# jamesli1618/Obj-GAN

Measured on AMD Instinct MI355X. Metric: G+D train-step images/sec at 256x256, batch 16 per GPU, higher is better.
Workload: dtype fp32 (fp16x2: operands as two fp16 pieces of x * 2^s on the fp16 MFMA); 1 GPU; stage3_256x256_full_GD_step: RNN_ENCODER+G_NET(3 stages)+PatD x3+ShpD x3+ObjSSD+ObjLSD(ROIAlign)+DAMSM+KL+Adam x9+EMA+IS-monitor; per_gpu_batch=16, global_batch=16, parallelism=dp1, fresh_batch_every_step=True

## Files before the change

### include/objgan_hip.h

```cpp
#ifndef OBJGAN_HIP_H
#define OBJGAN_HIP_H

#ifdef __cplusplus
extern "C" {
#endif

int objgan_roi_align_forward(const float* features, const float* rois, float* output,
                             int num_rois, int roi_cols, int channels, int height, int width,
                             int aligned_height, int aligned_width, float spatial_scale,
                             void* stream);
int objgan_roi_align_backward(const float* top_grad, const float* rois, float* bottom_grad,
                              int batch_size, int num_rois, int roi_cols, int channels,
                              int height, int width, int aligned_height, int aligned_width,
                              float spatial_scale, void* stream);

long objgan_roi_align_backward_ws_floats(int batch_size, int num_rois, int channels, int height, int width,
                                         int aligned_height, int aligned_width);
int objgan_roi_align_backward_ordered(const float* top_grad, const float* rois, float* bottom_grad,
                                      int batch_size, int num_rois, int roi_cols, int channels,
                                      int height, int width, int aligned_height, int aligned_width,
                                      float spatial_scale, float* ws, long ws_floats, void* stream);
int objgan_avgpool2s1_forward(const float* in, float* out, long planes, int ih, int iw, void* stream);
int objgan_avgpool2s1_backward(const float* grad_out, float* grad_in, long planes, int ih, int iw,
                               void* stream);

long objgan_conv_packed_floats(int M, int C, int T);
int objgan_conv_bank_layout(int N, int C, int H, int W, int M, int Tg, int PH, int PW, int act, int math);
int objgan_conv_igemm(const float* x, const float* w, const float* bias, float* y, float* wt,
                      int N, int C, int H, int W, int upsample, int pad_mode,
                      int Cout, int Cin, int Torig, int transpose,
                      int Tg, const int* dh, const int* dw, const int* src_tap,
                      int PH, int PW, int stride,
                      int OHf, int OWf, int osh, int osw, int ooh, int oow,
                      int act, int y_prezeroed, int wt_packed, int math, float* ring, const float* xmax, float* ymax,
                      float* ws, long ws_floats, void* stream);
int objgan_absmax_partials(const float* x, long n, float* out1024, void* stream);
long objgan_h2_records_floats(int N, int C, long HW);
int objgan_h2_records(const float* x, const float* xmax1024, void* rec, int N, int C, long HW, void* stream);
long objgan_conv_igemm_ws_floats(int N, int C, int H, int W, int upsample, int pad_mode,
                                 int Cout, int Cin, int Torig, int transpose, int Tg,
                                 int PH, int PW, int stride, int OHf, int OWf, int osh, int osw,
                                 int act, int y_prezeroed, int math, int ring);
int objgan_reflect_ring_fold(const float* ring, float* y, long planes, int H, int W, void* stream);
long objgan_conv_dgrad_s2_phases_ws_floats(int N, int Cout, int OH, int OW, int math);
long objgan_conv_dgrad_s2_thin_floats(int Cout, int Cin);
int objgan_conv_pack_job_thin_phase(void* job, const float* w, float* wt, int Cout, int Cin, int phase);
int objgan_conv_dgrad_s2_thin(const float* dy, const float* w, float* dx, float* wt, int N, int Cout, int OH, int OW,
                              int Cin, int wt_packed, void* stream);
int objgan_conv_dgrad_s2_phases(const float* x, const float* w, float* y, float* wt,
                                int N, int Cout, int OH, int OW, int Cin, int Torig,
                                int Tg, const int* dh, const int* dw, const int* src_tap,
                                int PH, int PW, int wt_packed, int math, const float* xmax, float* ws, long ws_floats,
                                void* stream);
long objgan_conv_wgrad_ws_floats(int N, int Cin, int H, int W, int upsample, int pad_mode,
                                 int Cout, int OH, int OW, int ksize, int stride, int pad, int math);
int objgan_conv_wgrad(const float* x, const float* dy, float* dw,
                      int N, int Cin, int H, int W, int upsample, int pad_mode,
                      int Cout, int OH, int OW, int ksize, int stride, int pad, int math,
                      int accumulate, const float* xmax, const float* dymax, float* ws, long ws_floats, void* stream);
int objgan_conv_wgrad_rec_ok(int N, int Cin, int H, int W, int Cout, int OH, int OW, int ksize);
long objgan_nhwc_bf16_floats(int N, int C, long HW);
int objgan_nhwc_bf16(const float* x, float* out, int N, int C, long HW, void* stream);
int objgan_conv_wgrad_bfb_ok(int N, int Cin, int H, int W, int Cout, int OH, int OW, int ksize);

int objgan_lstm_bidir_forward(const float* table, const long* captions, const int* lens,
                              const float* wt_ih, const float* wt_hh, const float* b_ih, const float* b_hh,
                              float* out, float* hn, int B, int L, int Lout, int I, int H, int ntoken,
                              void* stream);

long objgan_norm_ws_floats(int N, int C, int HW, int per_channel);
int objgan_norm_forward(const float* x, float* y, const float* residual,
                        const float* gamma, const float* beta,
                        float* running_mean, float* running_var,
                        float* sums, float* mean, float* rstd,
                        int N, int C, int HW, int per_channel, int mode,
                        float eps, float momentum, float* amax, void* stream);
int objgan_norm_amax_supported(int N, int C, int HW, int per_channel, int affine);
int objgan_norm_apply(const float* x, float* y, const float* residual, const float* gamma, const float* beta,
                      const float* mean, const float* rstd, int N, int C, int HW, int per_channel, int mode,
                      void* stream);
int objgan_norm_backward(const float* x, const float* dy, const float* mean, const float* rstd,
                         const float* gamma, const float* beta, float* bsums,
                         float* dx, float* dgamma, float* dbeta,
                         int N, int C, int HW, int per_channel, int mode, float* amax, void* stream);
int objgan_act_backward(const float* dy, const float* y, float* dz, long total, int kind, float* amax, void* stream);
long objgan_channel_sum_ws_floats(int N, int C, int HW);
int objgan_channel_sum(const float* x, float* out, int N, int C, int HW, float* ws, void* stream);

int objgan_attn_general_forward(const float* x, const float* src, const unsigned char* mask,
                                float* wc, float* attn, int B, int idf, int Q, int L, void* stream);
long objgan_attn_general_backward_ws_floats(int B, int idf, int Q, int L);
int objgan_attn_general_backward(const float* x, const float* src, const float* attn,
                                 const float* dwc, const float* dattn, float* dx, float* dsrc,
                                 int B, int idf, int Q, int L, float* ws, void* stream);
int objgan_attn_bu_forward(const float* tgt, const float* ctx1, const float* src,
                           const unsigned char* mask, float* wc, float* attn,
                           int B, int d2, int idf, int R, int L, int normalize, float eps,
                           void* stream);
int objgan_attn_bu_backward(const float* dwc, const float* attn, float* dsrc,
                            int B, int idf, int R, int L, void* stream);
int objgan_masked_max_forward(const float* f, const float* m, float* out, int B, int num, int R,
                              int P, long m_stride_b, long m_stride_r, long m_stride_c, void* stream);
long objgan_masked_max_backward_ws_floats(int B, int num, int R, int P);
int objgan_masked_max_backward(const float* f, const float* m, const float* dout, float* df,
                               int B, int num, int R, int P, long m_stride_b, long m_stride_r,
                               long m_stride_c, float* ws, void* stream);
int objgan_softmax_strided_forward(const float* x, float* y, long outer, int dim, long inner,
                                   float scale, const int* lens, int nlens,
                                   const unsigned char* rowvalid, void* stream);
int objgan_softmax_strided_backward(const float* y, const float* dy, float* dx, long outer, int dim,
                                    long inner, float scale, void* stream);

int objgan_bilinear_forward(const float* x, float* y, long planes, int ih, int iw, int oh, int ow,
                            void* stream);
int objgan_bilinear_backward(const float* dy, float* dx, long planes, int ih, int iw, int oh, int ow,
                             void* stream);
int objgan_sum2x2(const float* dy, float* dx, long planes, int h, int w, void* stream);
int objgan_reflect_fold(const float* dxp, float* dx, long planes, int h, int w, void* stream);
int objgan_bce_const_forward(const float* p, float* out, int n, float t, void* stream);
int objgan_bce_const_backward(const float* p, const float* g, float* dp, int n, float t, void* stream);
int objgan_conv_pack_job_bytes();
int objgan_conv_pack_job(void* job, const float* w, float* wt, int N, int C, int H, int W, int Cout, int Cin,
                         int Torig, int transpose, int Tg, const int* src_tap, int PH, int PW, int act, int math);
int objgan_conv_pack_job_phase(void* job, const float* w, float* wt, int Cout, int Cin, int Torig, int Tg,
                               const int* src_tap_phase, int phase, int math);
int objgan_conv_pack_jobs_run(const void* jobs_dev, int njobs, void* stream);
int objgan_bmm_strided(const float* A, const float* B, float* C, int batch, int M, int N, int K,
                       long sab, long sam, long sak, long sbb, long sbk, long sbn,
                       long scb, long scm, long scn, void* stream);
int objgan_lift_taps_forward(const float* z, const float* bias, float* y, float* scratch, int N, int Mo, int h,
                             int w, int SH, int SW, const int* ci0, const int* ci1, const float* cl1,
                             const int* ri0, const int* ri1, const float* rl1, void* stream);
int objgan_lift_taps_backward(const float* dy, float* dz, float* scratch, int N, int Mo, int h, int w, int SH,
                              int SW, const int* roff, const int* ridx, const float* rwt, const int* coff,
                              const int* cidx, const float* cwt, void* stream);
int objgan_pool2d_forward(const float* x, float* y, int* idx, long planes, int H, int W, int OH, int OW,
                          int k, int s, int p, int mode, void* stream);
int objgan_pool2d_backward(const float* dy, const int* idx, float* dx, long planes, int H, int W, int OH,
                           int OW, int k, int s, int p, int mode, void* stream);
int objgan_adam_step(float* p, const float* g, float* m, float* v, long n, double lr, double beta1,
                     double beta2, double eps, int step, float grad_scale, void* stream);
int objgan_adam_step_gated(float* p, const float* g, float* m, float* v, long n, double lr, double beta1,
                           double beta2, double eps, double* state, const float* flag, float* coef,
                           float grad_scale, void* stream);
int objgan_ema_update(float* avg, const float* p, long n, float decay, float one_minus_decay,
                      void* stream);

int objgan_resize_pil_kmax(int max_in, int S);
int objgan_resize_pil_rgb8(const unsigned char* src, const long* offs, const int* hs, const int* ws, int B,
                           int Hmax, int kmax, int S, int* coef_scratch, unsigned char* tmp_scratch, float* out,
                           void* stream);

long objgan_jpeg_desc_bytes(void);
long objgan_jpeg_seg_bytes(void);
int objgan_jpeg_parse(const unsigned char* file, long nbytes, void* desc_out);
long objgan_jpeg_plan(void* descs, int n, const long* file_offsets, const long* out_offsets, const int* nsegs);
int objgan_jpeg_decode(const unsigned char* files, const void* descs_host, const void* descs_dev, int n,
                       unsigned char* out, void* ws, long ws_bytes, const void* index_in, void* index_out, void* stream);

int objgan_mask_resize(const double* src, int count, int n, int nsizes, const int* sizes, double* const* out,
                       const int* ntaps, const double* taps, void* stream);

int objgan_bilinear_halfpixel_forward(const float* x, float* y, int N, int C, int H, int W, int OH, int OW,
                                      const float* scale, const float* shift, void* stream);
int objgan_moments_accumulate(const float* x, int rows, int D, double* sum, double* outer, void* stream);
int objgan_moments_finalize(const double* sum, const double* outer, long n, int D, double* mu, double* sigma,
                            void* stream);

long objgan_snapshot_ws_doubles(int nvis, int T, int a, int vis);
int objgan_snapshot_blend_table(unsigned char* table65536);
int objgan_snapshot_grid(const float* imgs, const float* lr_imgs, const float* attn, const int* counts, const double* M,
                         const unsigned char* strip, unsigned char* out, double* ws, long ws_doubles,
                         int nvis, int T, int a, int vis, int H, int W, int LH, int LW,
                         int max_word_num, int font_max, int per_panel_norm, void* stream);

int objgan_prof_enable(int on);
int objgan_prof_collect(double* ms, double* flops, long* count);
int objgan_prof_dump(float* ms, double* flops, int* meta, int max_records, int* n_out);

#ifdef __cplusplus
}
#endif
#endif
```

### obj-gan_amd/csrc/lift_stem.hip

```cpp
#include "common.h"

struct AxisFwd { const int* i0; const int* i1; const float* l1; };
struct AxisBwd { const int* off; const int* idx; const float* wt; };

#define LIFT_MAXE 8

__global__ __launch_bounds__(256) void lift_cols_fwd_kernel(const float* __restrict__ z, float* __restrict__ F,
                                                            long total, int Mo, int h, int w, int SW, AxisFwd t) {
    for (long e = (long)blockIdx.x * blockDim.x + threadIdx.x; e < total; e += (long)gridDim.x * blockDim.x) {
        const int ow = (int)(e % SW);
        long r = e / SW;
        const int qh = (int)(r % h);
        const long n = r / h;
        int i0[3], i1[3];
        float l1[3];
#pragma unroll
        for (int dw = 0; dw < 3; ++dw) { i0[dw] = t.i0[dw * SW + ow]; i1[dw] = t.i1[dw * SW + ow]; l1[dw] = t.l1[dw * SW + ow]; }
        const long hw = (long)h * w;
        const float* zn = z + n * 9 * Mo * hw + (long)qh * w;
        float* Fn = F + (n * 3 * Mo * h + qh) * (long)SW + ow;
        for (int dh = 0; dh < 3; ++dh)
            for (int co = 0; co < Mo; ++co) {
                float acc = 0.f;
#pragma unroll
                for (int dw = 0; dw < 3; ++dw) {
                    const float* zp = zn + ((dh * 3 + dw) * Mo + co) * hw;
                    acc += (1.0f - l1[dw]) * zp[i0[dw]] + l1[dw] * zp[i1[dw]];
                }
                Fn[(long)(dh * Mo + co) * h * SW] = acc;
            }
    }
}

__global__ __launch_bounds__(256) void lift_rows_fwd_kernel(const float* __restrict__ F, const float* __restrict__ bias,
                                                            float* __restrict__ y, long total, int Mo, int h,
                                                            int SH, int SW, AxisFwd t) {
    for (long e = (long)blockIdx.x * blockDim.x + threadIdx.x; e < total; e += (long)gridDim.x * blockDim.x) {
        const int ow = (int)(e % SW);
        long r = e / SW;
        const int oh = (int)(r % SH);
        const long n = r / SH;
        long o0[3], o1[3];
        float l1[3];
#pragma unroll
        for (int dh = 0; dh < 3; ++dh) {
            o0[dh] = (long)t.i0[dh * SH + oh] * SW; o1[dh] = (long)t.i1[dh * SH + oh] * SW; l1[dh] = t.l1[dh * SH + oh];
        }
        const long plane = (long)h * SW;
        const float* Fn = F + n * 3 * Mo * plane + ow;
        float* yn = y + (n * Mo * SH + oh) * (long)SW + ow;
        for (int co = 0; co < Mo; ++co) {
            float acc = bias ? bias[co] : 0.f;
#pragma unroll
            for (int dh = 0; dh < 3; ++dh) {
                const float* fp = Fn + (dh * Mo + co) * plane;
                acc += (1.0f - l1[dh]) * fp[o0[dh]] + l1[dh] * fp[o1[dh]];
            }
            yn[(long)co * SH * SW] = acc;
        }
    }
}

__global__ __launch_bounds__(256) void lift_rows_bwd_kernel(const float* __restrict__ dy, float* __restrict__ dF,
                                                            long total, int Mo, int h, int SH, int SW, AxisBwd t) {
    for (long e = (long)blockIdx.x * blockDim.x + threadIdx.x; e < total; e += (long)gridDim.x * blockDim.x) {
        const int ow = (int)(e % SW);
        long r = e / SW;
        const int qh = (int)(r % h);
        const long n = r / h;
        const float* gn = dy + n * Mo * (long)SH * SW + ow;
        float* dn = dF + (n * 3 * Mo * h + qh) * (long)SW + ow;
        for (int dh = 0; dh < 3; ++dh) {
            const int b = t.off[dh * (h + 1) + qh];
            const int cnt = min(t.off[dh * (h + 1) + qh + 1] - b, LIFT_MAXE);
            long of[LIFT_MAXE];
            float wv[LIFT_MAXE];
#pragma unroll
            for (int k = 0; k < LIFT_MAXE; ++k) {
                const bool on = k < cnt;
                of[k] = on ? (long)t.idx[b + k] * SW : 0;
                wv[k] = on ? t.wt[b + k] : 0.f;
            }
            for (int co = 0; co < Mo; ++co) {
                const float* gp = gn + (long)co * SH * SW;
                float acc = 0.f;
#pragma unroll
                for (int k = 0; k < LIFT_MAXE; ++k) acc += wv[k] * gp[of[k]];
                dn[(long)(dh * Mo + co) * h * SW] = acc;
            }
        }
    }
}

__global__ __launch_bounds__(256) void lift_cols_bwd_kernel(const float* __restrict__ dF, float* __restrict__ dz,
                                                            long total, int Mo, int h, int w, int SW, AxisBwd t) {
    for (long e = (long)blockIdx.x * blockDim.x + threadIdx.x; e < total; e += (long)gridDim.x * blockDim.x) {
        const int qw = (int)(e % w);
        long r = e / w;
        const int qh = (int)(r % h);
        const long n = r / h;
        const long hw = (long)h * w;
        const float* fn = dF + (n * 3 * Mo * h + qh) * (long)SW;
        float* zn = dz + n * 9 * Mo * hw + (long)qh * w + qw;
        for (int dw = 0; dw < 3; ++dw) {
            const int b = t.off[dw * (w + 1) + qw];
            const int cnt = min(t.off[dw * (w + 1) + qw + 1] - b, LIFT_MAXE);
            int of[LIFT_MAXE];
            float wv[LIFT_MAXE];
#pragma unroll
            for (int k = 0; k < LIFT_MAXE; ++k) {
                const bool on = k < cnt;
                of[k] = on ? t.idx[b + k] : 0;
                wv[k] = on ? t.wt[b + k] : 0.f;
            }
            for (int dh = 0; dh < 3; ++dh)
                for (int co = 0; co < Mo; ++co) {
                    const float* fp = fn + (long)(dh * Mo + co) * h * SW;
                    float acc = 0.f;
#pragma unroll
                    for (int k = 0; k < LIFT_MAXE; ++k) acc += wv[k] * fp[of[k]];
                    zn[((dh * 3 + dw) * Mo + co) * hw] = acc;
                }
        }
    }
}

extern "C" {

int objgan_lift_taps_forward(const float* z, const float* bias, float* y, float* scratch, int N, int Mo, int h,
                             int w, int SH, int SW, const int* ci0, const int* ci1, const float* cl1,
                             const int* ri0, const int* ri1, const float* rl1, void* stream) {
    OG_ENTRY();
    if (N <= 0 || Mo <= 0) return OG_OK;
    if (h < 1 || w < 1 || SH < 2 || SW < 2 || !scratch) return OG_BAD_ARGS;
    const long t1 = (long)N * h * SW, t2 = (long)N * SH * SW;
    AxisFwd tc = {ci0, ci1, cl1}, trw = {ri0, ri1, rl1};
    hipLaunchKernelGGL(lift_cols_fwd_kernel, dim3(og_stream_grid(t1, 256)), dim3(256), 0, (hipStream_t)stream,
                       z, scratch, t1, Mo, h, w, SW, tc);
    hipLaunchKernelGGL(lift_rows_fwd_kernel, dim3(og_stream_grid(t2, 256)), dim3(256), 0, (hipStream_t)stream,
                       (const float*)scratch, bias, y, t2, Mo, h, SH, SW, trw);
    return og_launch_status();
}

int objgan_lift_taps_backward(const float* dy, float* dz, float* scratch, int N, int Mo, int h, int w, int SH,
                              int SW, const int* roff, const int* ridx, const float* rwt, const int* coff,
                              const int* cidx, const float* cwt, void* stream) {
    OG_ENTRY();
    if (N <= 0 || Mo <= 0) return OG_OK;
    if (h < 1 || w < 1 || SH < 2 || SW < 2 || !scratch) return OG_BAD_ARGS;
    const long t1 = (long)N * h * SW, t2 = (long)N * h * w;
    AxisBwd trw = {roff, ridx, rwt}, tc = {coff, cidx, cwt};
    hipLaunchKernelGGL(lift_rows_bwd_kernel, dim3(og_stream_grid(t1, 256)), dim3(256), 0, (hipStream_t)stream,
                       dy, scratch, t1, Mo, h, SH, SW, trw);
    hipLaunchKernelGGL(lift_cols_bwd_kernel, dim3(og_stream_grid(t2, 256)), dim3(256), 0, (hipStream_t)stream,
                       (const float*)scratch, dz, t2, Mo, h, w, SW, tc);
    return og_launch_status();
}

}
```

### obj-gan_amd/objgan_hip/_lib.py

```python
import ctypes
import os

from . import build as _build

_c_int = ctypes.c_int
_c_long = ctypes.c_long
_c_float = ctypes.c_float
_c_double = ctypes.c_double
_ptr = ctypes.c_void_p

SIGNATURES = {
    "objgan_roi_align_forward": [_ptr, _ptr, _ptr, _c_int, _c_int, _c_int, _c_int, _c_int, _c_int, _c_int, _c_float, _ptr],
    "objgan_roi_align_backward": [_ptr, _ptr, _ptr, _c_int, _c_int, _c_int, _c_int, _c_int, _c_int, _c_int, _c_int, _c_float, _ptr],
    "objgan_roi_align_backward_ordered": [_ptr, _ptr, _ptr, _c_int, _c_int, _c_int, _c_int, _c_int, _c_int, _c_int, _c_int,
                                          _c_float, _ptr, _c_long, _ptr],
    "objgan_avgpool2s1_forward": [_ptr, _ptr, _c_long, _c_int, _c_int, _ptr],
    "objgan_avgpool2s1_backward": [_ptr, _ptr, _c_long, _c_int, _c_int, _ptr],
    "objgan_conv_igemm": [_ptr, _ptr, _ptr, _ptr, _ptr,
                          _c_int, _c_int, _c_int, _c_int, _c_int, _c_int,
                          _c_int, _c_int, _c_int, _c_int,
                          _c_int, _ptr, _ptr, _ptr,
                          _c_int, _c_int, _c_int,
                          _c_int, _c_int, _c_int, _c_int, _c_int, _c_int,
                          _c_int, _c_int, _c_int, _c_int, _ptr, _ptr, _ptr, _ptr, _c_long, _ptr],
    "objgan_absmax_partials": [_ptr, _c_long, _ptr, _ptr],
    "objgan_h2_records": [_ptr, _ptr, _ptr, _c_int, _c_int, _c_long, _ptr],
    "objgan_reflect_ring_fold": [_ptr, _ptr, _c_long, _c_int, _c_int, _ptr],
    "objgan_conv_dgrad_s2_phases": [_ptr, _ptr, _ptr, _ptr, _c_int, _c_int, _c_int, _c_int, _c_int, _c_int,
                                    _c_int, _ptr, _ptr, _ptr, _c_int, _c_int, _c_int, _c_int, _ptr, _ptr, _c_long, _ptr],
    "objgan_conv_wgrad": [_ptr, _ptr, _ptr, _c_int, _c_int, _c_int, _c_int, _c_int, _c_int,
                          _c_int, _c_int, _c_int, _c_int, _c_int, _c_int, _c_int, _c_int, _ptr, _ptr, _ptr, _c_long, _ptr],
    "objgan_lstm_bidir_forward": [_ptr, _ptr, _ptr, _ptr, _ptr, _ptr, _ptr, _ptr, _ptr,
                                  _c_int, _c_int, _c_int, _c_int, _c_int, _c_int, _ptr],
    "objgan_norm_forward": [_ptr, _ptr, _ptr, _ptr, _ptr, _ptr, _ptr, _ptr, _ptr, _ptr,
                            _c_int, _c_int, _c_int, _c_int, _c_int, _c_float, _c_float, _ptr, _ptr],
    "objgan_norm_amax_supported": [_c_int] * 5,
    "objgan_norm_apply": [_ptr, _ptr, _ptr, _ptr, _ptr, _ptr, _ptr, _c_int, _c_int, _c_int, _c_int, _c_int, _ptr],
    "objgan_norm_backward": [_ptr, _ptr, _ptr, _ptr, _ptr, _ptr, _ptr, _ptr, _ptr, _ptr,
                             _c_int, _c_int, _c_int, _c_int, _c_int, _ptr, _ptr],
    "objgan_act_backward": [_ptr, _ptr, _ptr, _c_long, _c_int, _ptr, _ptr],
    "objgan_channel_sum": [_ptr, _ptr, _c_int, _c_int, _c_int, _ptr, _ptr],
    "objgan_attn_general_forward": [_ptr, _ptr, _ptr, _ptr, _ptr, _c_int, _c_int, _c_int, _c_int, _ptr],
    "objgan_attn_general_backward": [_ptr, _ptr, _ptr, _ptr, _ptr, _ptr, _ptr, _c_int, _c_int, _c_int, _c_int, _ptr, _ptr],
    "objgan_attn_bu_forward": [_ptr, _ptr, _ptr, _ptr, _ptr, _ptr, _c_int, _c_int, _c_int, _c_int, _c_int, _c_int, _c_float, _ptr],
    "objgan_attn_bu_backward": [_ptr, _ptr, _ptr, _c_int, _c_int, _c_int, _c_int, _ptr],
    "objgan_masked_max_forward": [_ptr, _ptr, _ptr, _c_int, _c_int, _c_int, _c_int, _c_long, _c_long, _c_long, _ptr],
    "objgan_masked_max_backward": [_ptr, _ptr, _ptr, _ptr, _c_int, _c_int, _c_int, _c_int, _c_long, _c_long, _c_long, _ptr, _ptr],
    "objgan_softmax_strided_forward": [_ptr, _ptr, _c_long, _c_int, _c_long, _c_float, _ptr, _c_int, _ptr, _ptr],
    "objgan_softmax_strided_backward": [_ptr, _ptr, _ptr, _c_long, _c_int, _c_long, _c_float, _ptr],
    "objgan_bilinear_forward": [_ptr, _ptr, _c_long, _c_int, _c_int, _c_int, _c_int, _ptr],
    "objgan_bilinear_backward": [_ptr, _ptr, _c_long, _c_int, _c_int, _c_int, _c_int, _ptr],
    "objgan_bilinear_halfpixel_forward": [_ptr, _ptr, _c_int, _c_int, _c_int, _c_int, _c_int, _c_int, _ptr, _ptr, _ptr],
    "objgan_moments_accumulate": [_ptr, _c_int, _c_int, _ptr, _ptr, _ptr],
    "objgan_moments_finalize": [_ptr, _ptr, _c_long, _c_int, _ptr, _ptr, _ptr],
    "objgan_sum2x2": [_ptr, _ptr, _c_long, _c_int, _c_int, _ptr],
    "objgan_reflect_fold": [_ptr, _ptr, _c_long, _c_int, _c_int, _ptr],
    "objgan_conv_pack_job_bytes": [],
    "objgan_conv_pack_job": [_ptr, _ptr, _ptr, _c_int, _c_int, _c_int, _c_int, _c_int, _c_int, _c_int, _c_int,
                             _c_int, _ptr, _c_int, _c_int, _c_int, _c_int],
    "objgan_conv_pack_job_phase": [_ptr, _ptr, _ptr, _c_int, _c_int, _c_int, _c_int, _ptr, _c_int, _c_int],
    "objgan_conv_pack_job_thin_phase": [_ptr, _ptr, _ptr, _c_int, _c_int, _c_int],
    "objgan_conv_dgrad_s2_thin": [_ptr, _ptr, _ptr, _ptr, _c_int, _c_int, _c_int, _c_int, _c_int, _c_int, _ptr],
    "objgan_conv_pack_jobs_run": [_ptr, _c_int, _ptr],
    "objgan_bce_const_forward": [_ptr, _ptr, _c_int, _c_float, _ptr],
    "objgan_bce_const_backward": [_ptr, _ptr, _ptr, _c_int, _c_float, _ptr],
    "objgan_bmm_strided": [_ptr, _ptr, _ptr, _c_int, _c_int, _c_int, _c_int] + [_c_long] * 9 + [_ptr],
    "objgan_lift_taps_forward": [_ptr, _ptr, _ptr, _ptr, _c_int, _c_int, _c_int, _c_int, _c_int, _c_int,
                                 _ptr, _ptr, _ptr, _ptr, _ptr, _ptr, _ptr],
    "objgan_lift_taps_backward": [_ptr, _ptr, _ptr, _c_int, _c_int, _c_int, _c_int, _c_int, _c_int,
                                  _ptr, _ptr, _ptr, _ptr, _ptr, _ptr, _ptr],
    "objgan_pool2d_forward": [_ptr, _ptr, _ptr, _c_long, _c_int, _c_int, _c_int, _c_int, _c_int, _c_int, _c_int, _c_int, _ptr],
    "objgan_pool2d_backward": [_ptr, _ptr, _ptr, _c_long, _c_int, _c_int, _c_int, _c_int, _c_int, _c_int, _c_int, _c_int, _ptr],
    "objgan_adam_step": [_ptr, _ptr, _ptr, _ptr, _c_long, _c_double, _c_double, _c_double, _c_double, _c_int, _c_float, _ptr],
    "objgan_adam_step_gated": [_ptr, _ptr, _ptr, _ptr, _c_long, _c_double, _c_double, _c_double, _c_double,
                               _ptr, _ptr, _ptr, _c_float, _ptr],
    "objgan_ema_update": [_ptr, _ptr, _c_long, _c_float, _c_float, _ptr],
    "objgan_resize_pil_kmax": [_c_int, _c_int],
    "objgan_resize_pil_rgb8": [_ptr, _ptr, _ptr, _ptr, _c_int, _c_int, _c_int, _c_int, _ptr, _ptr, _ptr, _ptr],
    "objgan_mask_resize": [_ptr, _c_int, _c_int, _c_int, _ptr, _ptr, _ptr, _ptr, _ptr],
    "objgan_jpeg_parse": [ctypes.c_char_p, _c_long, _ptr],
    "objgan_jpeg_decode": [_ptr, _ptr, _ptr, _c_int, _ptr, _ptr, _c_long, _ptr, _ptr, _ptr],
    "objgan_snapshot_blend_table": [_ptr],
    "objgan_snapshot_grid": [_ptr, _ptr, _ptr, _ptr, _ptr, _ptr, _ptr, _ptr, _c_long] + [_c_int] * 11 + [_ptr],
    "objgan_prof_enable": [_c_int],
    "objgan_conv_bank_layout": [_c_int] * 10,
    "objgan_conv_wgrad_rec_ok": [_c_int] * 8,
    "objgan_conv_wgrad_bfb_ok": [_c_int] * 8,
    "objgan_nhwc_bf16": [_ptr, _ptr, _c_int, _c_int, _c_long, _ptr],
    "objgan_prof_collect": [_ptr, _ptr, _ptr],
    "objgan_prof_dump": [_ptr, _ptr, _ptr, _c_int, _ptr],
}
LONG_RETURN = {"objgan_conv_packed_floats": [_c_int, _c_int, _c_int],
               "objgan_conv_igemm_ws_floats": [_c_int] * 22,
               "objgan_conv_wgrad_ws_floats": [_c_int] * 13,
               "objgan_conv_dgrad_s2_phases_ws_floats": [_c_int] * 5,
               "objgan_conv_dgrad_s2_thin_floats": [_c_int, _c_int],
               "objgan_h2_records_floats": [_c_int, _c_int, _c_long],
               "objgan_nhwc_bf16_floats": [_c_int, _c_int, _c_long],
               "objgan_norm_ws_floats": [_c_int] * 4,
               "objgan_attn_general_backward_ws_floats": [_c_int] * 4,
               "objgan_masked_max_backward_ws_floats": [_c_int] * 4,
               "objgan_channel_sum_ws_floats": [_c_int] * 3,
               "objgan_roi_align_backward_ws_floats": [_c_int] * 7,
               "objgan_snapshot_ws_doubles": [_c_int] * 4,
               "objgan_jpeg_desc_bytes": [],
               "objgan_jpeg_seg_bytes": [],
               "objgan_jpeg_plan": [_ptr, _c_int, _ptr, _ptr, _ptr]}

_LIB = None


class ObjganHipError(RuntimeError):
    pass


def lib_path():
    return _build.LIB_PATH


def load(build_if_missing=True):
    global _LIB
    if _LIB is not None:
        return _LIB
    path = lib_path()
    if not os.path.exists(path):
        if not build_if_missing:
            raise ObjganHipError("libobjgan_hip.so not built: run `python -c 'import __graft_entry__ as g; g.build()'`")
        _build.build(verbose=False)
    import torch
    lib = ctypes.CDLL(path)
    for name, argtypes in SIGNATURES.items():
        fn = getattr(lib, name)
        fn.argtypes = argtypes
        fn.restype = _c_int
    for name, argtypes in LONG_RETURN.items():
        fn = getattr(lib, name)
        fn.argtypes = argtypes
        fn.restype = _c_long
    _LIB = lib
    return lib


def call(name, *args):
    rc = getattr(load(), name)(*args)
    if rc == 1:
        return
    if rc == 0:
        raise ObjganHipError("%s: invalid arguments (returned 0)" % name)
    raise ObjganHipError("%s: HIP launch failed (hipError %d)" % (name, -rc))
```

### obj-gan_amd/objgan_hip/ops.py

```python
import ctypes
import math

import os

import torch

from . import _lib

_F32 = torch.float32


def _p(t):
    return None if t is None else ctypes.c_void_p(t.data_ptr())


def _stream():
    return ctypes.c_void_p(torch._C._cuda_getCurrentRawStream(torch._C._cuda_getDevice()))


def _chk(*tensors):
    for t in tensors:
        if t is None:
            continue
        if not t.is_cuda:
# ... 1660 lines not shown
    for k, S in enumerate(sizes):
        if S < n:
            w = _gaussian_taps((n / float(S) - 1.0) / 2.0)
            if len(w) > 17:
                raise _lib.ObjganHipError("resize_masks: shrinking %d -> %d is outside the table (radius <= 8)" % (n, S))
            ntaps.append(len(w))
            taps[17 * k:17 * k + len(w)] = [float(v) for v in w]
        else:
            ntaps.append(0)
    outp = (ctypes.c_void_p * len(sizes))(*[o.data_ptr() for o in outs])
    _lib.call("objgan_mask_resize", _p(src), count, n, len(sizes), _iarr(sizes), outp, _iarr(ntaps),
              (ctypes.c_double * len(taps))(*taps), _stream())
    return outs


_EXPAND = {}


def expansion_matrix(a, vis, sigma=20.0):
    import numpy as np
    a, vis = int(a), int(vis)

    def mirror(i, n):
        if n == 1:
            return 0
        i = i % (2 * n - 2)
        return i if i < n else 2 * n - 2 - i

    Z = np.zeros((vis, a), np.float64)
    for o in range(vis):
        c = (o + 0.5) * (a / float(vis)) - 0.5
        if a == 1:
            c = 0.0
        elif c < 0:
            c = -c
        i = int(np.floor(c))
        f = c - i
        Z[o, mirror(i, a)] += 1.0 - f
        Z[o, mirror(i + 1, a)] += f
    w = _gaussian_taps(sigma)
    r = len(w) // 2
    G = np.zeros((vis, vis), np.float64)
    for o in range(vis):
        for k in range(-r, r + 1):
            G[o, mirror(o + k, vis)] += w[k + r]
    return G.dot(Z)


def _expansion_matrix_dev(a, vis, device):
    key = (int(a), int(vis), str(device))
    m = _EXPAND.get(key)
    if m is None:
        m = _EXPAND[key] = torch.from_numpy(expansion_matrix(a, vis)).pin_memory().to(device, non_blocking=True)
    return m


def paste_blend_table():
    import numpy as np
    table = np.empty((256, 256), np.uint8)
    _lib.call("objgan_snapshot_blend_table", ctypes.c_void_p(table.ctypes.data))
    return table


def snapshot_grid(imgs, attn_maps, att_sze, text_strip, lr_imgs=None, max_word_num=12, font_max=50, nvis=8,
                  per_panel_norm=False):
    as_list = isinstance(attn_maps, (list, tuple))
    _chk(imgs, lr_imgs, *(attn_maps if as_list else (attn_maps,)))
    if not (torch.is_tensor(text_strip) and text_strip.is_cuda and text_strip.dtype == torch.uint8):
        raise _lib.ObjganHipError("snapshot_grid: text_strip is a uint8 tensor on the GPU (there is no CPU path)")
    if imgs.dim() != 4 or imgs.shape[1] != 3 or (lr_imgs is not None and (lr_imgs.dim() != 4 or lr_imgs.shape[1] != 3)):
        raise _lib.ObjganHipError("snapshot_grid: images are [B, 3, h, w]")
    B, a, nvis, font_max, mw = int(imgs.shape[0]), int(att_sze), int(nvis), int(font_max), int(max_word_num)
    H, W = int(imgs.shape[2]), int(imgs.shape[3])
    vis = a * 16 if a == 17 else H
    if (not 1 <= nvis <= B or (len(attn_maps) if as_list else attn_maps.shape[0]) < nvis
            or (lr_imgs is not None and lr_imgs.shape[0] < nvis)):
        raise _lib.ObjganHipError("snapshot_grid: nvis = %d images wanted, batch of %d" % (nvis, B))
    counts = None
    if as_list:
        per = [m.detach().reshape(-1, a, a) for m in attn_maps[:nvis]]
        sizes = [int(m.shape[0]) for m in per]
        attn = torch.zeros((nvis, max(sizes + [1]), a, a), dtype=_F32, device=imgs.device)
        for i, m in enumerate(per):
            attn[i, :sizes[i]].copy_(m)
        if min(sizes) < 1:
            raise _lib.ObjganHipError("snapshot_grid: an image without attention maps")
        counts = torch.tensor(sizes, dtype=torch.int32).pin_memory().to(imgs.device, non_blocking=True)
    else:
        attn = _c(attn_maps.detach()).reshape(int(attn_maps.shape[0]), -1, a, a)
    T = int(attn.shape[1])
    ratio = vis // a
    if ratio < 1 or (ratio == 1 and vis != a) or not 1 <= T <= 1023:
        raise _lib.ObjganHipError("snapshot_grid: %d maps of %d x %d cannot be drawn into %d x %d panels" % (T, a, a, vis, vis))
    width = (mw + 2) * (vis + 2)
    if tuple(text_strip.shape) != (nvis * font_max, width, 3):
        raise _lib.ObjganHipError("snapshot_grid: text_strip is %s, expected %s"
                                  % (tuple(text_strip.shape), (nvis * font_max, width, 3)))
    imgs = _c(imgs.detach())
    lr = _c(lr_imgs.detach()) if lr_imgs is not None else None
    LH, LW = (int(lr.shape[2]), int(lr.shape[3])) if lr is not None else (0, 0)
    M = _expansion_matrix_dev(a, vis, imgs.device) if ratio > 1 else None
    nws = _q("objgan_snapshot_ws_doubles", nvis, T, a, vis)
    ws = torch.empty(nws, dtype=torch.float64, device=imgs.device)
    out = torch.empty((nvis * (font_max + 2 * vis), width, 3), dtype=torch.uint8, device=imgs.device)
    _lib.call("objgan_snapshot_grid", _p(imgs), _p(lr), _p(attn), _p(counts), _p(M), _p(_c(text_strip)), _p(out), _p(ws), nws,
              nvis, T, a, vis, H, W, LH, LW, mw, font_max, 1 if per_panel_norm else 0, _stream())
    return out


_LIFT_TABLES = {}


def _lift_axis_tables(n_in, n_out, device):
    key = (n_in, n_out, str(device))
    ent = _LIFT_TABLES.get(key)
    if ent is not None:
        return ent
    import numpy as np
    scale = np.float32(n_in - 1) / np.float32(n_out - 1) if n_out > 1 else np.float32(0)
    i0s, i1s, l1s, offs, idxs, wts = [], [], [], [], [], []
    base = 0
    for d in (-1, 0, 1):
        r = np.arange(n_out, dtype=np.int64) + d
        r = np.where(r < 0, -r, r)
        r = np.where(r >= n_out, 2 * (n_out - 1) - r, r)
        src = (scale * r.astype(np.float32)).astype(np.float32)
        i0 = np.minimum(src.astype(np.int32), n_in - 1)
        i1 = i0 + (i0 < n_in - 1)
        l1 = (src - i0.astype(np.float32)).astype(np.float32)
        l0 = (np.float32(1.0) - l1).astype(np.float32)
        i0s.append(i0); i1s.append(i1); l1s.append(l1)
        q = np.concatenate([i0, i1]).astype(np.int64)
        o = np.concatenate([np.arange(n_out), np.arange(n_out)])
        wv = np.concatenate([l0, l1])
        order = np.lexsort((o, q))
        q, o, wv = q[order], o[order], wv[order]
        off = np.zeros(n_in + 1, np.int64)
        np.add.at(off, q + 1, 1)
        off = np.cumsum(off) + base
        base = int(off[-1])
        offs.append(off); idxs.append(o); wts.append(wv)
    def t(arrays, dt, flat=False):
        a = np.concatenate(arrays) if flat else np.stack(arrays)
        return torch.from_numpy(np.ascontiguousarray(a.astype(dt))).to(device)
    longest = max(int((o[1:] - o[:-1]).max()) for o in offs)
    if longest > 8:
        raise _lib.ObjganHipError("lift_stem_conv: lift factor %d -> %d too large for the adjoint kernel" % (n_in, n_out))
    ent = (t(i0s, np.int32), t(i1s, np.int32), t(l1s, np.float32),
           t(offs, np.int32), t(idxs, np.int32, True), t(wts, np.float32, True))
    _LIFT_TABLES[key] = ent
    return ent


class _LiftTapsFn(torch.autograd.Function):
    @staticmethod
    def forward(ctx, z, bias, SH, SW):
        _chk(z, bias)
        z = _c(z)
        N, C9, h, w = z.shape
        Mo = C9 // 9
        rows = _lift_axis_tables(h, SH, z.device)
        cols = _lift_axis_tables(w, SW, z.device)
        y = torch.empty((N, Mo, SH, SW), dtype=_F32, device=z.device)
        scratch = torch.empty(N * 3 * Mo * h * SW, dtype=_F32, device=z.device)
        _lib.call("objgan_lift_taps_forward", _p(z), _p(bias), _p(y), _p(scratch), N, Mo, h, w, SH, SW,
                  _p(cols[0]), _p(cols[1]), _p(cols[2]), _p(rows[0]), _p(rows[1]), _p(rows[2]), _stream())
        ctx.geom = (N, Mo, h, w, SH, SW)
        ctx.has_bias = bias is not None
        return y

    @staticmethod
    def backward(ctx, dy):
        N, Mo, h, w, SH, SW = ctx.geom
        dy = _c(dy)
        _chk(dy)
        dz = db = None
        if ctx.needs_input_grad[0]:
            rows = _lift_axis_tables(h, SH, dy.device)
            cols = _lift_axis_tables(w, SW, dy.device)
            dz = torch.empty((N, 9 * Mo, h, w), dtype=_F32, device=dy.device)
            scratch = torch.empty(N * 3 * Mo * h * SW, dtype=_F32, device=dy.device)
            _lib.call("objgan_lift_taps_backward", _p(dy), _p(dz), _p(scratch), N, Mo, h, w, SH, SW,
                      _p(rows[3]), _p(rows[4]), _p(rows[5]), _p(cols[3]), _p(cols[4]), _p(cols[5]), _stream())
        if ctx.has_bias and ctx.needs_input_grad[1]:
            db = torch.empty(Mo, dtype=_F32, device=dy.device)
            _channel_sum(dy, db, N, Mo, SH * SW)
        return dz, db, None, None


def lift_stem_conv(seg, w, bias, size):
    Mo, C = w.shape[0], w.shape[1]
    if w.shape[2] != 3 or w.shape[3] != 3:
        raise _lib.ObjganHipError("lift_stem_conv: 3x3 filter bank expected")
    w9 = w.permute(2, 3, 0, 1).reshape(9 * Mo, C, 1, 1).contiguous()
    w9._og_nocache = True
    z = conv2d(seg, w9)
    return _LiftTapsFn.apply(z, bias, int(size), int(size))


def lstm_bidir_forward(table, captions, lens, wt_ih, wt_hh, b_ih, b_hh, max_len):
    _chk(table, wt_ih, wt_hh, b_ih, b_hh)
    if not captions.is_cuda or captions.dtype != torch.int64:
        raise _lib.ObjganHipError("lstm: captions must be an int64 tensor on the GPU")
    captions = _c(captions)
    lens = _c(lens.to(device=captions.device, dtype=torch.int32))
    B, L = captions.shape
    I, G = wt_ih.shape[1], wt_ih.shape[2]
    H = G // 4
    out = torch.empty((B, 2 * H, int(max_len)), dtype=_F32, device=captions.device)
    hn = torch.empty((B, 2 * H), dtype=_F32, device=captions.device)
    _lib.call("objgan_lstm_bidir_forward", _p(table), _p(captions), _p(lens), _p(wt_ih), _p(wt_hh),
              _p(b_ih), _p(b_hh), _p(out), _p(hn), B, L, int(max_len), I, H, table.shape[0], _stream())
    return out, hn


def adam_step_(p, g, m, v, lr, beta1, beta2, eps, step, grad_scale=1.0, n=None):
    _chk(p, g, m, v)
    n = p.numel() if n is None else int(n)
    _lib.call("objgan_adam_step", _p(p), _p(g), _p(m), _p(v), n, float(lr), float(beta1),
              float(beta2), float(eps), int(step), float(grad_scale), _stream())


def adam_step_gated_(p, g, m, v, lr, beta1, beta2, eps, state, flag, coef, grad_scale=1.0, n=None):
    _chk(p, g, m, v, flag, coef)
    if not state.is_cuda or state.dtype != torch.float64 or state.numel() < 3:
        raise _lib.ObjganHipError("adam_step_gated_: state must be 3 float64 values on the GPU")
    n = p.numel() if n is None else int(n)
    _lib.call("objgan_adam_step_gated", _p(p), _p(g), _p(m), _p(v), n, float(lr), float(beta1),
              float(beta2), float(eps), _p(state), _p(flag), _p(coef), float(grad_scale), _stream())


def ema_update_(avg, p, decay):
    _chk(avg, p)
    _lib.call("objgan_ema_update", _p(avg), _p(p), p.numel(), float(decay), float(1.0 - decay), _stream())
```

Measured before the change: 120.4 images/sec.

## Fuse lift-stem separable interpolation passes into single LDS-tiled kernels

Adds fused forward and backward kernels for the lift-stem tap interpolation. Each block keeps the intermediate column-interpolated band in LDS, so the two-pass scheme no longer writes and rereads a global scratch buffer. The backward kernel also computes the gradient's absolute max inline for fp16 scaling, replacing a separate reduction. By default only the backward path is fused; the forward fused path needs OBJGAN_LIFT_FUSED=2. This trades large LDS use and 512-thread blocks, which may limit occupancy, for less memory traffic and fewer launches.

```diff
diff --git a/include/objgan_hip.h b/include/objgan_hip.h
--- a/include/objgan_hip.h
+++ b/include/objgan_hip.h
@@ -134,6 +134,13 @@
 int objgan_lift_taps_backward(const float* dy, float* dz, float* scratch, int N, int Mo, int h, int w, int SH,
                               int SW, const int* roff, const int* ridx, const float* rwt, const int* coff,
                               const int* cidx, const float* cwt, void* stream);
+int objgan_lift_taps_fused_ok(int h, int w, int SH, int SW);
+int objgan_lift_taps_forward_fused(const float* z, const float* bias, float* y, int N, int Mo, int h, int w, int SH,
+                                   int SW, const int* ci0, const int* ci1, const float* cl1, const int* ri0,
+                                   const int* ri1, const float* rl1, void* stream);
+int objgan_lift_taps_backward_fused(const float* dy, float* dz, int N, int Mo, int h, int w, int SH, int SW,
+                                    const int* roff, const int* ridx, const float* rwt, const int* coff,
+                                    const int* cidx, const float* cwt, float* amax, void* stream);
 int objgan_pool2d_forward(const float* x, float* y, int* idx, long planes, int H, int W, int OH, int OW,
                           int k, int s, int p, int mode, void* stream);
 int objgan_pool2d_backward(const float* dy, const int* idx, float* dx, long planes, int H, int W, int OH,
diff --git a/obj-gan_amd/csrc/lift_stem.hip b/obj-gan_amd/csrc/lift_stem.hip
--- a/obj-gan_amd/csrc/lift_stem.hip
+++ b/obj-gan_amd/csrc/lift_stem.hip
@@ -125,6 +125,202 @@
     }
 }
 
+#define LIFT_FT 512
+#define LIFT_TH 32
+#define LIFT_TQ 8
+#define LIFT_LDS_MAX 63488
+
+static inline int lift_span(int n_src, int n_dst, int T) {
+    if (n_dst < 2 || n_src < 2) return n_src;
+    const long s = ((long)(T + 1) * (n_src - 1)) / (n_dst - 1) + 5;
+    return (int)(s < n_src ? s : n_src);
+}
+static inline int lift_fwd_rows(int h, int SH) { return lift_span(h, SH, LIFT_TH); }
+static inline int lift_bwd_band(int h, int SH, int SW, int* DB) {
+    for (int tq = LIFT_TQ; tq >= 1; tq >>= 1) {
+        const int db = lift_span(SH, h, tq);
+        if ((long)(db + tq) * SW * 4 <= LIFT_LDS_MAX) { *DB = db; return tq; }
+    }
+    return 0;
+}
+static inline int lift_fused_ok(int h, int w, int SH, int SW) {
+    int db;
+    return h >= 1 && w >= 1 && SH >= 2 && SW >= 2 && w <= LIFT_FT && SW <= LIFT_FT &&
+           (long)lift_fwd_rows(h, SH) * SW * 4 <= LIFT_LDS_MAX && lift_bwd_band(h, SH, SW, &db) > 0;
+}
+
+__device__ __forceinline__ int lift_wave_min(int v) {
+#pragma unroll
+    for (int o = 32; o > 0; o >>= 1) v = min(v, __shfl_xor(v, o, 64));
+    return v;
+}
+__device__ __forceinline__ int lift_wave_max(int v) {
+#pragma unroll
+    for (int o = 32; o > 0; o >>= 1) v = max(v, __shfl_xor(v, o, 64));
+    return v;
+}
+
+__global__ __launch_bounds__(LIFT_FT) void lift_fwd_fused_kernel(const float* __restrict__ z, const float* __restrict__ bias,
+                                                                 float* __restrict__ y, int Mo, int h, int w, int SH, int SW,
+                                                                 int RB, int ntr, AxisFwd tc, AxisFwd tr) {
+    extern __shared__ float Fs[];
+    int b = blockIdx.x;
+    const int rt = b % ntr; b /= ntr;
+    const int co = b % Mo;
+    const long n = b / Mo;
+    const int oh0 = rt * LIFT_TH, nh = min(LIFT_TH, SH - oh0);
+    __shared__ int s_i0[3 * LIFT_TH], s_i1[3 * LIFT_TH];
+    __shared__ float s_l1[3 * LIFT_TH];
+    if (threadIdx.x < 3 * LIFT_TH) {
+        const int dh = threadIdx.x / LIFT_TH, r = threadIdx.x % LIFT_TH;
+        const bool in = r < nh;
+        s_i0[threadIdx.x] = in ? tr.i0[dh * SH + oh0 + r] : h - 1;
+        s_i1[threadIdx.x] = in ? tr.i1[dh * SH + oh0 + r] : 0;
+        s_l1[threadIdx.x] = in ? tr.l1[dh * SH + oh0 + r] : 0.f;
+    }
+    __syncthreads();
+    int lo = h - 1, hi = 0;
+    for (int e = threadIdx.x & 63; e < 3 * LIFT_TH; e += 64) { lo = min(lo, s_i0[e]); hi = max(hi, s_i1[e]); }
+    lo = max(lift_wave_min(lo), 0);
+    hi = min(lift_wave_max(hi), h - 1);
+    const int R = min(hi - lo + 1, RB);
+    const int G = LIFT_FT / SW, c = threadIdx.x % SW, g = threadIdx.x / SW;
+    const bool on = g < G;
+    int i0[3], i1[3];
+    float l1[3];
+#pragma unroll
+    for (int dw = 0; dw < 3; ++dw) { i0[dw] = tc.i0[dw * SW + c]; i1[dw] = tc.i1[dw * SW + c]; l1[dw] = tc.l1[dw * SW + c]; }
+    const long hw = (long)h * w;
+    const float* zn = z + (n * 9 * Mo + co) * hw + (long)lo * w;
+    const float bv = bias ? bias[co] : 0.f;
+    float acc[LIFT_TH];
+#pragma unroll
+    for (int k = 0; k < LIFT_TH; ++k) acc[k] = bv;
+    for (int dh = 0; dh < 3; ++dh) {
+        if (on) {
+#pragma unroll 2
+            for (int r = g; r < R; r += G) {
+                float a = 0.f;
+#pragma unroll
+                for (int dw = 0; dw < 3; ++dw) {
+                    const float* zp = zn + (long)((dh * 3 + dw) * Mo) * hw + (long)r * w;
+                    a = __fadd_rn(a, __fmaf_rn(1.0f - l1[dw], zp[i0[dw]], __fmul_rn(l1[dw], zp[i1[dw]])));
+                }
+                Fs[r * SW + c] = a;
+            }
+        }
+        __syncthreads();
+        if (on) {
+#pragma unroll
+            for (int k = 0; k < LIFT_TH; ++k) {
+                const int r = g + k * G;
+                if (r < nh) {
+                    const int a0 = min(max(s_i0[dh * LIFT_TH + r] - lo, 0), R - 1);
+                    const int a1 = min(max(s_i1[dh * LIFT_TH + r] - lo, 0), R - 1);
+                    const float lr = s_l1[dh * LIFT_TH + r];
+                    const float fa = Fs[a0 * SW + c], tb = __fmul_rn(lr, Fs[a1 * SW + c]);
+                    acc[k] = __fadd_rn(acc[k], dh == 0 ? __fadd_rn(__fmul_rn(1.0f - lr, fa), tb) : __fmaf_rn(1.0f - lr, fa, tb));
+                }
+            }
+        }
+        __syncthreads();
+    }
+    if (on) {
+        float* yn = y + ((n * Mo + co) * SH + oh0) * (long)SW + c;
+#pragma unroll
+        for (int k = 0; k < LIFT_TH; ++k) {
+            const int r = g + k * G;
+            if (r < nh) yn[(long)r * SW] = acc[k];
+        }
+    }
+}
+
+__global__ __launch_bounds__(LIFT_FT) void lift_bwd_fused_kernel(const float* __restrict__ dy, float* __restrict__ dz,
+                                                                 float* __restrict__ amax, int Mo, int h, int w, int SH,
+                                                                 int SW, int TQ, int DB, int ntq, AxisBwd tr, AxisBwd tc) {
+    extern __shared__ float sm[];
+    __shared__ float red[LIFT_FT / 64];
+    float* gL = sm;
+    float* fL = sm + DB * SW;
+    int b = blockIdx.x;
+    const int rt = b % ntq; b /= ntq;
+    const int co = b % Mo;
+    const long n = b / Mo;
+    const int qh0 = rt * TQ, nq = min(TQ, h - qh0);
+    __shared__ int s_idx[3 * LIFT_TQ * LIFT_MAXE];
+    __shared__ float s_wt[3 * LIFT_TQ * LIFT_MAXE];
+    if (threadIdx.x < 3 * LIFT_TQ * LIFT_MAXE) {
+        const int dh = threadIdx.x / (LIFT_TQ * LIFT_MAXE), q = (threadIdx.x / LIFT_MAXE) % LIFT_TQ, k = threadIdx.x % LIFT_MAXE;
+        bool in = q < nq;
+        int e0 = 0;
+        if (in) {
+            e0 = tr.off[dh * (h + 1) + qh0 + q];
+            in = k < tr.off[dh * (h + 1) + qh0 + q + 1] - e0;
+        }
+        s_idx[threadIdx.x] = in ? tr.idx[e0 + k] : -1;
+        s_wt[threadIdx.x] = in ? tr.wt[e0 + k] : 0.f;
+    }
+    __syncthreads();
+    int lo = SH, hi = -1;
+    for (int e = threadIdx.x & 63; e < 3 * LIFT_TQ * LIFT_MAXE; e += 64) {
+        const int v = s_idx[e];
+        if (v >= 0) { lo = min(lo, v); hi = max(hi, v); }
+    }
+    lo = max(lift_wave_min(lo), 0);
+    hi = min(lift_wave_max(hi), SH - 1);
+    const int D = max(min(hi - lo + 1, DB), 0);
+    const float* gp = dy + ((n * Mo + co) * SH + lo) * (long)SW;
+#pragma unroll 4
+    for (int i = threadIdx.x; i < D * SW; i += LIFT_FT) gL[i] = gp[i];
+    __syncthreads();
+    const int G = LIFT_FT / SW, c = threadIdx.x % SW, g = threadIdx.x / SW;
+    const int G2 = LIFT_FT / w, qw = threadIdx.x % w, g2 = threadIdx.x / w;
+    const long hw = (long)h * w;
+    float* zn = dz + (n * 9 * Mo + co) * hw + (long)qh0 * w + qw;
+    int of[3][LIFT_MAXE];
+    float wv[3][LIFT_MAXE];
+#pragma unroll
+    for (int dw = 0; dw < 3; ++dw) {
+        const int e0 = tc.off[dw * (w + 1) + qw];
+        const int cnt = tc.off[dw * (w + 1) + qw + 1] - e0;
+#pragma unroll
+        for (int k = 0; k < LIFT_MAXE; ++k) {
+            const bool in = k < cnt;
+            of[dw][k] = in ? min(max(tc.idx[e0 + k], 0), SW - 1) : 0;
+            wv[dw][k] = in ? tc.wt[e0 + k] : 0.f;
+        }
+    }
+    float m = 0.f;
+    for (int dh = 0; dh < 3; ++dh) {
+        if (g < G)
+            for (int q = g; q < nq; q += G) {
+                const int e = (dh * LIFT_TQ + q) * LIFT_MAXE;
+                float a = 0.f;
+#pragma unroll
+                for (int k = 0; k < LIFT_MAXE; ++k) {
+                    const int v = s_idx[e + k];
+                    if (v >= 0) a = __fmaf_rn(s_wt[e + k], gL[min(max(v - lo, 0), D - 1) * SW + c], a);
+                }
+                fL[q * SW + c] = a;
+            }
+        __syncthreads();
+        if (g2 < G2)
+            for (int q = g2; q < nq; q += G2) {
+                const float* fp = fL + q * SW;
+#pragma unroll
+                for (int dw = 0; dw < 3; ++dw) {
+                    float a = 0.f;
+#pragma unroll
+                    for (int k = 0; k < LIFT_MAXE; ++k) a = __fmaf_rn(wv[dw][k], fp[of[dw][k]], a);
+                    zn[(long)((dh * 3 + dw) * Mo) * hw + (long)q * w] = a;
+                    m = fmaxf(m, fabsf(a));
+                }
+            }
+        __syncthreads();
+    }
+    if (amax) og_amax_atomic(og_block_max(m, red), amax, blockIdx.x);
+}
+
 extern "C" {
 
 int objgan_lift_taps_forward(const float* z, const float* bias, float* y, float* scratch, int N, int Mo, int h,
@@ -157,4 +353,37 @@
     return og_launch_status();
 }
 
-}
+int objgan_lift_taps_fused_ok(int h, int w, int SH, int SW) { return lift_fused_ok(h, w, SH, SW) ? 1 : 0; }
+
+int objgan_lift_taps_forward_fused(const float* z, const float* bias, float* y, int N, int Mo, int h, int w, int SH,
+                                   int SW, const int* ci0, const int* ci1, const float* cl1, const int* ri0,
+                                   const int* ri1, const float* rl1, void* stream) {
+    OG_ENTRY();
+    if (N <= 0 || Mo <= 0) return OG_OK;
+    if (!lift_fused_ok(h, w, SH, SW)) return OG_BAD_ARGS;
+    const int RB = lift_fwd_rows(h, SH), ntr = og_cdiv(SH, LIFT_TH);
+    const long grid = (long)N * Mo * ntr;
+    if (grid > 0x7fffffffL) return OG_BAD_ARGS;
+    AxisFwd tc = {ci0, ci1, cl1}, trw = {ri0, ri1, rl1};
+    hipLaunchKernelGGL(lift_fwd_fused_kernel, dim3((unsigned)grid), dim3(LIFT_FT), (size_t)RB * SW * 4,
+                       (hipStream_t)stream, z, bias, y, Mo, h, w, SH, SW, RB, ntr, tc, trw);
+    return og_launch_status();
+}
+
+int objgan_lift_taps_backward_fused(const float* dy, float* dz, int N, int Mo, int h, int w, int SH, int SW,
+                                    const int* roff, const int* ridx, const float* rwt, const int* coff,
+                                    const int* cidx, const float* cwt, float* amax, void* stream) {
+    OG_ENTRY();
+    if (N <= 0 || Mo <= 0) return OG_OK;
+    if (!lift_fused_ok(h, w, SH, SW)) return OG_BAD_ARGS;
+    int DB = 0;
+    const int TQ = lift_bwd_band(h, SH, SW, &DB), ntq = og_cdiv(h, TQ);
+    const long grid = (long)N * Mo * ntq;
+    if (grid > 0x7fffffffL) return OG_BAD_ARGS;
+    AxisBwd trw = {roff, ridx, rwt}, tc = {coff, cidx, cwt};
+    hipLaunchKernelGGL(lift_bwd_fused_kernel, dim3((unsigned)grid), dim3(LIFT_FT), (size_t)(DB + TQ) * SW * 4,
+                       (hipStream_t)stream, dy, dz, amax, Mo, h, w, SH, SW, TQ, DB, ntq, trw, tc);
+    return og_launch_status();
+}
+
+}
diff --git a/obj-gan_amd/objgan_hip/_lib.py b/obj-gan_amd/objgan_hip/_lib.py
--- a/obj-gan_amd/objgan_hip/_lib.py
+++ b/obj-gan_amd/objgan_hip/_lib.py
@@ -69,6 +69,11 @@
                                  _ptr, _ptr, _ptr, _ptr, _ptr, _ptr, _ptr],
     "objgan_lift_taps_backward": [_ptr, _ptr, _ptr, _c_int, _c_int, _c_int, _c_int, _c_int, _c_int,
                                   _ptr, _ptr, _ptr, _ptr, _ptr, _ptr, _ptr],
+    "objgan_lift_taps_fused_ok": [_c_int] * 4,
+    "objgan_lift_taps_forward_fused": [_ptr, _ptr, _ptr, _c_int, _c_int, _c_int, _c_int, _c_int, _c_int,
+                                       _ptr, _ptr, _ptr, _ptr, _ptr, _ptr, _ptr],
+    "objgan_lift_taps_backward_fused": [_ptr, _ptr, _c_int, _c_int, _c_int, _c_int, _c_int, _c_int,
+                                        _ptr, _ptr, _ptr, _ptr, _ptr, _ptr, _ptr, _ptr],
     "objgan_pool2d_forward": [_ptr, _ptr, _ptr, _c_long, _c_int, _c_int, _c_int, _c_int, _c_int, _c_int, _c_int, _c_int, _ptr],
     "objgan_pool2d_backward": [_ptr, _ptr, _ptr, _c_long, _c_int, _c_int, _c_int, _c_int, _c_int, _c_int, _c_int, _c_int, _ptr],
     "objgan_adam_step": [_ptr, _ptr, _ptr, _ptr, _c_long, _c_double, _c_double, _c_double, _c_double, _c_int, _c_float, _ptr],
diff --git a/obj-gan_amd/objgan_hip/ops.py b/obj-gan_amd/objgan_hip/ops.py
--- a/obj-gan_amd/objgan_hip/ops.py
+++ b/obj-gan_amd/objgan_hip/ops.py
@@ -1836,6 +1836,13 @@
     return ent
 
 
+_LIFT_FUSED = {"on": _os.environ.get("OBJGAN_LIFT_FUSED", "1") != "0", "fwd": _os.environ.get("OBJGAN_LIFT_FUSED") == "2"}
+
+
+def _lift_fused(h, w, SH, SW, forward=False):
+    return _LIFT_FUSED["on"] and (_LIFT_FUSED["fwd"] or not forward) and _q("objgan_lift_taps_fused_ok", h, w, SH, SW) == 1
+
+
 class _LiftTapsFn(torch.autograd.Function):
     @staticmethod
     def forward(ctx, z, bias, SH, SW):
@@ -1846,9 +1853,13 @@
         rows = _lift_axis_tables(h, SH, z.device)
         cols = _lift_axis_tables(w, SW, z.device)
         y = torch.empty((N, Mo, SH, SW), dtype=_F32, device=z.device)
-        scratch = torch.empty(N * 3 * Mo * h * SW, dtype=_F32, device=z.device)
-        _lib.call("objgan_lift_taps_forward", _p(z), _p(bias), _p(y), _p(scratch), N, Mo, h, w, SH, SW,
-                  _p(cols[0]), _p(cols[1]), _p(cols[2]), _p(rows[0]), _p(rows[1]), _p(rows[2]), _stream())
+        if _lift_fused(h, w, SH, SW, forward=True):
+            _lib.call("objgan_lift_taps_forward_fused", _p(z), _p(bias), _p(y), N, Mo, h, w, SH, SW,
+                      _p(cols[0]), _p(cols[1]), _p(cols[2]), _p(rows[0]), _p(rows[1]), _p(rows[2]), _stream())
+        else:
+            scratch = torch.empty(N * 3 * Mo * h * SW, dtype=_F32, device=z.device)
+            _lib.call("objgan_lift_taps_forward", _p(z), _p(bias), _p(y), _p(scratch), N, Mo, h, w, SH, SW,
+                      _p(cols[0]), _p(cols[1]), _p(cols[2]), _p(rows[0]), _p(rows[1]), _p(rows[2]), _stream())
         ctx.geom = (N, Mo, h, w, SH, SW)
         ctx.has_bias = bias is not None
         return y
@@ -1863,9 +1874,16 @@
             rows = _lift_axis_tables(h, SH, dy.device)
             cols = _lift_axis_tables(w, SW, dy.device)
             dz = torch.empty((N, 9 * Mo, h, w), dtype=_F32, device=dy.device)
-            scratch = torch.empty(N * 3 * Mo * h * SW, dtype=_F32, device=dy.device)
-            _lib.call("objgan_lift_taps_backward", _p(dy), _p(dz), _p(scratch), N, Mo, h, w, SH, SW,
-                      _p(rows[3]), _p(rows[4]), _p(rows[5]), _p(cols[3]), _p(cols[4]), _p(cols[5]), _stream())
+            if _lift_fused(h, w, SH, SW):
+                am = _amax_zeroed(dy.device) if _amax_wanted(dz.numel()) else None
+                _lib.call("objgan_lift_taps_backward_fused", _p(dy), _p(dz), N, Mo, h, w, SH, SW, _p(rows[3]), _p(rows[4]),
+                          _p(rows[5]), _p(cols[3]), _p(cols[4]), _p(cols[5]), _p(am), _stream())
+                if am is not None:
+                    _amax_attach(dz, am)
+            else:
+                scratch = torch.empty(N * 3 * Mo * h * SW, dtype=_F32, device=dy.device)
+                _lib.call("objgan_lift_taps_backward", _p(dy), _p(dz), _p(scratch), N, Mo, h, w, SH, SW,
+                          _p(rows[3]), _p(rows[4]), _p(rows[5]), _p(cols[3]), _p(cols[4]), _p(cols[5]), _stream())
         if ctx.has_bias and ctx.needs_input_grad[1]:
             db = torch.empty(Mo, dtype=_F32, device=dy.device)
             _channel_sum(dy, db, N, Mo, SH * SW)
```

Result: no change. 121.2 images/sec (median of 6 runs) (+0.6%).
